# Audio-WestlakeU/FN-SSL

Measured on AMD Instinct MI355X. Metric: TF-frames/sec DP-IPD forward, 4-mic 257-bin x 300-frame, higher is better.
Workload: dtype f32; 1 GPU; BASELINE configs[1]: FN-SSL (online) DP-IPD forward, waveform->STFT->features->3x(full-band BiLSTM + narrow-band LSTM)->head; 32 utterances/GPU x 4 mics ('MM' = 6 pairs) x 257 bins x 300 frames, fp32; frame = one STFT frame of one utterance; stream_chunk_frames=0, utterances_per_gpu=32, global_batch=32, mics=4, pairs_per_utterance=6, frames=300, bins=257, parallelism=dp1 (utterance shards, no collective), chunk_pairs=0

## Files before the change

fn-ssl_amd/csrc/lstm_static4.h:

```cpp
#pragma once

#include "lstm_static.h"

#pragma clang fp contract(off)

namespace fnssl_lstm {

constexpr int static4_blocks_in_chunk(int qe, int chq, int nv0, int ns2, int ns) {
  int n = 0;
  for (int q = qe - chq + 1; q <= qe; ++q) {
    const bool x = q >= 1 && q <= nv0;
    const bool h = q >= 1 + nv0 + ns2 && q < 1 + nv0 + ns2 + ns;
    n += (x || h) ? 1 : 0;
  }
  return n;
}

template <int H, int NW, int NV0, int NS2, int CHQ, int PAD, int MODE, int XD = 4, bool PF4 = false>
__global__ void __launch_bounds__(NW * 64) lstm_static4_kernel(const LstmParams p) {
  FNSSL_GUARDED_KERNEL(p);
  constexpr int NS = H / 16, NP = NS / 4;
  constexpr int NB = NV0 + NS;
  constexpr bool HAS2 = (MODE & kHas2) != 0, SUM = (MODE & kSum) != 0;
  static_assert(!(MODE & kHas1) && HAS2 == (NS2 > 0) && NS % 4 == 0 && NS2 <= 1, "modes");
  constexpr int QPS = 1 + NV0 + NS2 + NS;
  constexpr int VQ = QPS + PAD;
  static_assert(VQ % CHQ == 0, "chunks must tile the (padded) slice quad");
  constexpr int CH = 16 * CHQ;
  constexpr int M = (CH + NW - 1) / NW;
  static_assert(PAD < CHQ, "a chunk of padding only would have no operand load to count the DMA by");
  extern __shared__ __attribute__((aligned(16))) char smem[];

  const WaveSeq<H, NW, 1, HAS2, SUM> pl(p);
  const int lane = pl.lane, w = pl.w;
  const rsrc_t rzero = __builtin_amdgcn_make_buffer_rsrc(const_cast<float*>(p.out), 0, 0, 0x00020000);

  const unsigned lds0 = (unsigned)(uintptr_t)smem;
  char* const lds_rd = smem + lane * 16;
  int dslot = 0, rslot = 0;
  int src_rec = 0;
  int src_vq = 0;
  auto issue_dma = [&]() {
#pragma unroll
    for (int m = 0; m < M; ++m) {
      const int r = w + m * NW;
      if (r < CH && src_vq * 16 + r < QPS * 16) {
        const unsigned soff = (unsigned)(src_rec + r) * 1024u;
        const unsigned ld = lds0 + (unsigned)(dslot * CH + r) * 1024u;
        asm volatile("s_mov_b32 m0, %2\n\ts_nop 0\n\tbuffer_load_dwordx4 %0, %1, %3 offen lds" ::"v"(pl.vlane), "s"(pl.rw),
                     "s"(__builtin_amdgcn_readfirstlane(ld)), "s"(__builtin_amdgcn_readfirstlane(soff))
                     : "memory");
      }
    }
    dslot ^= 1;
    src_vq += CHQ;
    src_rec += CH;
    if (src_vq == VQ) {
      src_vq = 0;
      src_rec -= PAD * 16;
      if (src_rec == NP * QPS * 16) src_rec = 0;
    }
  };
  issue_dma();
  asm volatile("s_waitcnt vmcnt(0)\n\ts_barrier" ::: "memory");
  issue_dma();
  const char* cb = lds_rd;
  auto rec = [&](auto ql, int j) { return *reinterpret_cast<const v4f*>(cb + decltype(ql)::value * 16384 + j * 1024); };
  v4f a0 = rec(ic<0>{}, 0), a1 = rec(ic<0>{}, 1);

  const v4f zero4 = v4f{0.f, 0.f, 0.f, 0.f};
  v4f acc[4][4];

  auto ring_step = [&](auto qi_c) {
    constexpr int QL = decltype(qi_c)::value % CHQ;
    if constexpr (QL + 1 < CHQ) {
      a0 = rec(ic<QL + 1>{}, 0);
      a1 = rec(ic<QL + 1>{}, 1);
    }
  };
  auto ring_end = [&](auto qi_c) {
    constexpr int QI = decltype(qi_c)::value, QL = QI % CHQ;
    if constexpr (QL + 1 == CHQ) {
      constexpr int K = static4_blocks_in_chunk(QI, CHQ, NV0, NS2, NS);
#ifdef FNSSL_BUILD_ABLATE
      asm volatile("s_waitcnt vmcnt(0)" ::: "memory");
#else
      if constexpr (K >= 3)
        asm volatile("s_waitcnt vmcnt(3)" ::: "memory");
      else if constexpr (K == 2)
        asm volatile("s_waitcnt vmcnt(2)" ::: "memory");
      else if constexpr (K == 1)
        asm volatile("s_waitcnt vmcnt(1)" ::: "memory");
      else
        asm volatile("s_waitcnt vmcnt(0)" ::: "memory");
#endif
      asm volatile("s_waitcnt lgkmcnt(0)\n\ts_barrier" ::: "memory");
      issue_dma();
      rslot ^= 1;
      cb = lds_rd + rslot * (CH * 1024);
      a0 = rec(ic<0>{}, 0);
      a1 = rec(ic<0>{}, 1);
    }
  };
#define SQUAD4(QI, B0, B1, B2, B3)                                                \
  do {                                                                            \
    const v4f a2_ = rec(ic<(QI) % CHQ>{}, 2), a3_ = rec(ic<(QI) % CHQ>{}, 3);     \
    __builtin_amdgcn_sched_barrier(0);                                            \
    MFMA4(acc[0], a0, B0);                                                        \
    MFMA4(acc[0], a1, B1);                                                        \
    const v4f b0_ = rec(ic<(QI) % CHQ>{}, 4), b1_ = rec(ic<(QI) % CHQ>{}, 5);     \
    __builtin_amdgcn_sched_barrier(0);                                            \
    MFMA4(acc[0], a2_, B2);                                                       \
    MFMA4(acc[0], a3_, B3);                                                       \
    const v4f b2_ = rec(ic<(QI) % CHQ>{}, 6), b3_ = rec(ic<(QI) % CHQ>{}, 7);     \
    __builtin_amdgcn_sched_barrier(0);                                            \
    MFMA4(acc[1], b0_, B0);                                                       \
    MFMA4(acc[1], b1_, B1);                                                       \
    const v4f c0_ = rec(ic<(QI) % CHQ>{}, 8), c1_ = rec(ic<(QI) % CHQ>{}, 9);     \
    __builtin_amdgcn_sched_barrier(0);                                            \
    MFMA4(acc[1], b2_, B2);                                                       \
    MFMA4(acc[1], b3_, B3);                                                       \
    const v4f c2_ = rec(ic<(QI) % CHQ>{}, 10), c3_ = rec(ic<(QI) % CHQ>{}, 11);   \
    __builtin_amdgcn_sched_barrier(0);                                            \
    MFMA4(acc[2], c0_, B0);                                                       \
    MFMA4(acc[2], c1_, B1);                                                       \
    const v4f d0_ = rec(ic<(QI) % CHQ>{}, 12), d1_ = rec(ic<(QI) % CHQ>{}, 13);   \
    __builtin_amdgcn_sched_barrier(0);                                            \
    MFMA4(acc[2], c2_, B2);                                                       \
    MFMA4(acc[2], c3_, B3);                                                       \
    const v4f d2_ = rec(ic<(QI) % CHQ>{}, 14), d3_ = rec(ic<(QI) % CHQ>{}, 15);   \
    __builtin_amdgcn_sched_barrier(0);                                            \
    MFMA4(acc[3], d0_, B0);                                                       \
    MFMA4(acc[3], d1_, B1);                                                       \
    ring_step(ic<(QI)>{});                                                        \
    __builtin_amdgcn_sched_barrier(0);                                            \
    MFMA4(acc[3], d2_, B2);                                                       \
    MFMA4(acc[3], d3_, B3);                                                       \
    ring_end(ic<(QI)>{});                                                         \
  } while (0)
#define SQUAD4_1(QI, B0)                                                                          \
  do {                                                                                            \
    const v4f b0_ = rec(ic<(QI) % CHQ>{}, 4), c0_ = rec(ic<(QI) % CHQ>{}, 8), d0_ = rec(ic<(QI) % CHQ>{}, 12); \
    MFMA4(acc[0], a0, B0);                                                                        \
    MFMA4(acc[1], b0_, B0);                                                                       \
    MFMA4(acc[2], c0_, B0);                                                                       \
    MFMA4(acc[3], d0_, B0);                                                                       \
    ring_step(ic<(QI)>{});                                                                        \
    ring_end(ic<(QI)>{});                                                                         \
  } while (0)

  OperandRing<XD, NV0, NS> ops;
  ops.prime(pl.rx0, pl.vo0, (pl.rev ? p.nsteps - 1 : 0) * pl.st0);

  for (int step = 0; step < p.nsteps; ++step) {
    const unsigned tt = pl.rev ? p.nsteps - 1 - step : step;
    const unsigned ttn = step + 1 < p.nsteps ? (pl.rev ? tt - 1 : tt + 1) : tt;
    const unsigned o0 = tt * pl.st0, o2 = tt * pl.st2, oo = tt * pl.sto, ok = tt * pl.stk;
    const unsigned op = (pl.rev ? tt + 1 : tt - 1) * pl.sto;
    const rsrc_t rh = step > 0 ? pl.ro : rzero;
    float xs2 = 0.f;
    if (NS2) xs2 = bld1(pl.rx2, pl.vo2, o2);

    for (int pr = 0; pr < NP; ++pr) {
      const int s0 = 4 * pr;
#ifdef FNSSL_BUILD_ABLATE
      const bool skip_ring = (p.ablate & 2) != 0;
#else
      constexpr bool skip_ring = false;
#endif
      v4f cprev = zero4, skipv = zero4;
      v4f cpf[PF4 ? 4 : 1], skf[PF4 ? 4 : 1];
      if constexpr (PF4) static_for<4>([&](auto s_) { cpf[s_.value] = zero4; skf[s_.value] = zero4; });
      const bool last = pr + 1 == NP;
      const unsigned nx = (last ? ttn : tt) * pl.st0;
      acc[0][0] = a0;
      acc[0][1] = a1;
      static_for<14>([&](auto j) {
        constexpr int J = decltype(j)::value + 2;
        acc[J / 4][J % 4] = rec(ic<0>{}, J);
      });
      ring_step(ic<0>{});
      ring_end(ic<0>{});
      static_for<NB>([&](auto bc) {
        constexpr int B = decltype(bc)::value;
        constexpr int QI = B < NV0 ? 1 + B : 1 + NS2 + B;
        if constexpr (NS2 > 0 && B == NV0) SQUAD4_1(1 + NV0, xs2);
        const v4f ob = ops.get(bc);
        if (!skip_ring) ops.request(bc, pl.rx0, pl.vo0, o0, nx, rh, pl.voo, op);
        if constexpr (!PF4 && B == NB - 4) {
          if (step > 0) cprev = bld4(pl.rc, pl.vlane, s0 * 1024);
          if (SUM) skipv = bld4(pl.rsk, pl.vok, ok + 64 * s0);
        }
        if constexpr (PF4 && B == NB - 3) {
          static_for<4>([&](auto s_) {
            constexpr int S = decltype(s_)::value;
            if (step > 0) cpf[S] = bld4(pl.rc, pl.vlane, (s0 + S) * 1024);
            if (SUM) skf[S] = bld4(pl.rsk, pl.vok, ok + 64 * (s0 + S));
          });
        }
        SQUAD4(QI, ob.x, ob.y, ob.z, ob.w);
      });
      static_for<PAD>([&](auto u) {
        ring_step(ic<QPS + decltype(u)::value>{});
        ring_end(ic<QPS + decltype(u)::value>{});
      });
      static_for<4>([&](auto sc) {
        constexpr int S = decltype(sc)::value;
        if constexpr (PF4) {
          cell_step(pl, acc[S], cpf[S], skf[S], (s0 + S) * 1024, oo + 64 * (s0 + S));
        } else {
          cell_step(pl, acc[S], cprev, skipv, (s0 + S) * 1024, oo + 64 * (s0 + S), [&] {
            if constexpr (S < 3) {
              if (step > 0) cprev = bld4(pl.rc, pl.vlane, (s0 + S + 1) * 1024);
              if (SUM) skipv = bld4(pl.rsk, pl.vok, ok + 64 * (s0 + S + 1));
            }
          });
        }
      });
    }
  }
  asm volatile("s_waitcnt vmcnt(0)" ::: "memory");
#undef SQUAD4
#undef SQUAD4_1
}

template <int H, int NW, int NV0, int NS2, int CHQ, int PAD, int MODE, int XD = 4, bool PF4 = false>
int launch_static4_k(const LstmParams& p, int nwg, const LaunchCtx& lc) {
  const size_t lds = (size_t)2 * CHQ * 16384;
  static_assert(2 * CHQ * 16384 <= 160 * 1024, "ring does not fit the LDS");
  return enqueue(lc, Kernel{lstm_static4_kernel<H, NW, NV0, NS2, CHQ, PAD, MODE, XD, PF4>, NW * 64, lds, "lstm_static4_kernel"}, nwg, p);
}

}
```

Baseline: 17780 frames/s.

## Interleave weight-ring DMA pieces between MFMA groups instead of bulk issue at chunk end

Instead of issuing all buffer_load-to-LDS pieces for the next weight chunk in one burst after the barrier, each piece is now placed at a compile-time-chosen MFMA group inside the first block quad of the current chunk. A constexpr schedule header computes piece placement and the matching vmcnt wait count per chunk, with static asserts to keep it consistent. Source and destination offsets become mostly compile-time with a wave-uniform base, and the step>0 branch on cell-state loads is replaced by a zero buffer descriptor. The intent is to hide DMA issue cost and spread memory traffic under MFMA work, at the risk of tighter wait counts and more scheduling constraints.

```diff
diff --git a/fn-ssl_amd/csrc/lstm_static4.h b/fn-ssl_amd/csrc/lstm_static4.h
--- a/fn-ssl_amd/csrc/lstm_static4.h
+++ b/fn-ssl_amd/csrc/lstm_static4.h
@@ -1,20 +1,11 @@
 #pragma once
 
 #include "lstm_static.h"
+#include "lstm_static4_sched.h"
 
 #pragma clang fp contract(off)
 
 namespace fnssl_lstm {
-
-constexpr int static4_blocks_in_chunk(int qe, int chq, int nv0, int ns2, int ns) {
-  int n = 0;
-  for (int q = qe - chq + 1; q <= qe; ++q) {
-    const bool x = q >= 1 && q <= nv0;
-    const bool h = q >= 1 + nv0 + ns2 && q < 1 + nv0 + ns2 + ns;
-    n += (x || h) ? 1 : 0;
-  }
-  return n;
-}
 
 template <int H, int NW, int NV0, int NS2, int CHQ, int PAD, int MODE, int XD = 4, bool PF4 = false>
 __global__ void __launch_bounds__(NW * 64) lstm_static4_kernel(const LstmParams p) {
@@ -29,6 +20,11 @@
   constexpr int CH = 16 * CHQ;
   constexpr int M = (CH + NW - 1) / NW;
   static_assert(PAD < CHQ, "a chunk of padding only would have no operand load to count the DMA by");
+  static_assert(M * NW == CH, "every wave issues every piece: the schedule has no wave-dependent piece");
+  constexpr Static4Shape SH{CHQ, NV0, NS2, NS, PAD, M};
+  constexpr int NC = VQ / CHQ;
+  static_assert(static4_schedule_ok(SH), "every chunk must place its M pieces and have a wait count");
+  constexpr unsigned SLOT = CH * 1024u;
   extern __shared__ __attribute__((aligned(16))) char smem[];
 
   const WaveSeq<H, NW, 1, HAS2, SUM> pl(p);
@@ -37,33 +33,35 @@
 
   const unsigned lds0 = (unsigned)(uintptr_t)smem;
   char* const lds_rd = smem + lane * 16;
-  int dslot = 0, rslot = 0;
-  int src_rec = 0;
-  int src_vq = 0;
-  auto issue_dma = [&]() {
-#pragma unroll
-    for (int m = 0; m < M; ++m) {
-      const int r = w + m * NW;
-      if (r < CH && src_vq * 16 + r < QPS * 16) {
-        const unsigned soff = (unsigned)(src_rec + r) * 1024u;
-        const unsigned ld = lds0 + (unsigned)(dslot * CH + r) * 1024u;
-        asm volatile("s_mov_b32 m0, %2\n\ts_nop 0\n\tbuffer_load_dwordx4 %0, %1, %3 offen lds" ::"v"(pl.vlane), "s"(pl.rw),
-                     "s"(__builtin_amdgcn_readfirstlane(ld)), "s"(__builtin_amdgcn_readfirstlane(soff))
-                     : "memory");
+  int rslot = 0;
+  const unsigned w_rec = (unsigned)w * 1024u;
+  constexpr unsigned PASS = QPS * 16384u;
+  auto dma_piece = [&](auto sc_c, auto m_c, unsigned src, unsigned dst) {
+    constexpr int SC = decltype(sc_c)::value, MI = decltype(m_c)::value;
+    constexpr int NVALID = static4_chunk_records(SH, SC);
+    if constexpr (MI * NW < NVALID) {
+      asm volatile("" : "+s"(src), "+s"(dst));
+      if constexpr (NVALID < MI * NW + NW) {
+        unsigned wc;
+        asm("s_min_u32 %0, %1, %2" : "=s"(wc) : "s"(w_rec), "s"((unsigned)(NVALID - 1 - MI * NW) * 1024u) : "scc");
+        src = src - w_rec + wc;
       }
-    }
-    dslot ^= 1;
-    src_vq += CHQ;
-    src_rec += CH;
-    if (src_vq == VQ) {
-      src_vq = 0;
-      src_rec -= PAD * 16;
-      if (src_rec == NP * QPS * 16) src_rec = 0;
-    }
-  };
-  issue_dma();
+      const unsigned soff = src + (unsigned)(SC * CH + MI * NW) * 1024u;
+      const unsigned ld = dst + (unsigned)(MI * NW) * 1024u;
+      const unsigned vl = pl.vlane;
+      const rsrc_t rw = pl.rw;
+#pragma clang diagnostic push
+#pragma clang diagnostic ignored "-Winline-asm"
+      asm volatile("s_mov_b32 m0, %2\n\ts_nop 0\n\tbuffer_load_dwordx4 %0, %1, %3 offen lds" ::"v"(vl), "s"(rw), "s"(ld), "s"(soff)
+                   : "memory", "m0");
+#pragma clang diagnostic pop
+    }
+  };
+  int ring_pr = 0;
+  auto src_cur = [&] { return (unsigned)ring_pr * PASS + w_rec; };
+  auto src_nxt = [&] { return (ring_pr + 1 < NP ? (unsigned)(ring_pr + 1) * PASS : 0u) + w_rec; };
+  static_for<M>([&](auto m_c) { dma_piece(ic<0>{}, m_c, w_rec, lds0 + w_rec); });
   asm volatile("s_waitcnt vmcnt(0)\n\ts_barrier" ::: "memory");
-  issue_dma();
   const char* cb = lds_rd;
   auto rec = [&](auto ql, int j) { return *reinterpret_cast<const v4f*>(cb + decltype(ql)::value * 16384 + j * 1024); };
   v4f a0 = rec(ic<0>{}, 0), a1 = rec(ic<0>{}, 1);
@@ -81,11 +79,12 @@
   auto ring_end = [&](auto qi_c) {
     constexpr int QI = decltype(qi_c)::value, QL = QI % CHQ;
     if constexpr (QL + 1 == CHQ) {
-      constexpr int K = static4_blocks_in_chunk(QI, CHQ, NV0, NS2, NS);
+      constexpr int C = QI / CHQ, K = static4_wait_count(SH, C);
+      static_assert(static4_pieces_placed(SH, C) == M && K >= 0 && K <= 3, "schedule");
 #ifdef FNSSL_BUILD_ABLATE
       asm volatile("s_waitcnt vmcnt(0)" ::: "memory");
 #else
-      if constexpr (K >= 3)
+      if constexpr (K == 3)
         asm volatile("s_waitcnt vmcnt(3)" ::: "memory");
       else if constexpr (K == 2)
         asm volatile("s_waitcnt vmcnt(2)" ::: "memory");
@@ -95,47 +94,60 @@
         asm volatile("s_waitcnt vmcnt(0)" ::: "memory");
 #endif
       asm volatile("s_waitcnt lgkmcnt(0)\n\ts_barrier" ::: "memory");
-      issue_dma();
       rslot ^= 1;
       cb = lds_rd + rslot * (CH * 1024);
       a0 = rec(ic<0>{}, 0);
       a1 = rec(ic<0>{}, 1);
     }
   };
+  auto ring_dma = [&](auto qi_c, auto g_c) {
+    constexpr int QI = decltype(qi_c)::value, C = QI / CHQ, MI = static4_piece_at(SH, QI, decltype(g_c)::value);
+    if constexpr (MI >= 0) {
+      dma_piece(ic<(C + 1) % NC>{}, ic<MI>{}, C + 1 < NC ? src_cur() : src_nxt(), lds0 + (unsigned)(rslot ^ 1) * SLOT + w_rec);
+    }
+  };
 #define SQUAD4(QI, B0, B1, B2, B3)                                                \
   do {                                                                            \
     const v4f a2_ = rec(ic<(QI) % CHQ>{}, 2), a3_ = rec(ic<(QI) % CHQ>{}, 3);     \
     __builtin_amdgcn_sched_barrier(0);                                            \
     MFMA4(acc[0], a0, B0);                                                        \
     MFMA4(acc[0], a1, B1);                                                        \
+    ring_dma(ic<(QI)>{}, ic<0>{});                                                \
     const v4f b0_ = rec(ic<(QI) % CHQ>{}, 4), b1_ = rec(ic<(QI) % CHQ>{}, 5);     \
     __builtin_amdgcn_sched_barrier(0);                                            \
     MFMA4(acc[0], a2_, B2);                                                       \
     MFMA4(acc[0], a3_, B3);                                                       \
+    ring_dma(ic<(QI)>{}, ic<1>{});                                                \
     const v4f b2_ = rec(ic<(QI) % CHQ>{}, 6), b3_ = rec(ic<(QI) % CHQ>{}, 7);     \
     __builtin_amdgcn_sched_barrier(0);                                            \
     MFMA4(acc[1], b0_, B0);                                                       \
     MFMA4(acc[1], b1_, B1);                                                       \
+    ring_dma(ic<(QI)>{}, ic<2>{});                                                \
     const v4f c0_ = rec(ic<(QI) % CHQ>{}, 8), c1_ = rec(ic<(QI) % CHQ>{}, 9);     \
     __builtin_amdgcn_sched_barrier(0);                                            \
     MFMA4(acc[1], b2_, B2);                                                       \
     MFMA4(acc[1], b3_, B3);                                                       \
+    ring_dma(ic<(QI)>{}, ic<3>{});                                                \
     const v4f c2_ = rec(ic<(QI) % CHQ>{}, 10), c3_ = rec(ic<(QI) % CHQ>{}, 11);   \
     __builtin_amdgcn_sched_barrier(0);                                            \
     MFMA4(acc[2], c0_, B0);                                                       \
     MFMA4(acc[2], c1_, B1);                                                       \
+    ring_dma(ic<(QI)>{}, ic<4>{});                                                \
     const v4f d0_ = rec(ic<(QI) % CHQ>{}, 12), d1_ = rec(ic<(QI) % CHQ>{}, 13);   \
     __builtin_amdgcn_sched_barrier(0);                                            \
     MFMA4(acc[2], c2_, B2);                                                       \
     MFMA4(acc[2], c3_, B3);                                                       \
+    ring_dma(ic<(QI)>{}, ic<5>{});                                                \
     const v4f d2_ = rec(ic<(QI) % CHQ>{}, 14), d3_ = rec(ic<(QI) % CHQ>{}, 15);   \
     __builtin_amdgcn_sched_barrier(0);                                            \
     MFMA4(acc[3], d0_, B0);                                                       \
     MFMA4(acc[3], d1_, B1);                                                       \
+    ring_dma(ic<(QI)>{}, ic<6>{});                                                \
     ring_step(ic<(QI)>{});                                                        \
     __builtin_amdgcn_sched_barrier(0);                                            \
     MFMA4(acc[3], d2_, B2);                                                       \
     MFMA4(acc[3], d3_, B3);                                                       \
+    ring_dma(ic<(QI)>{}, ic<7>{});                                                \
     ring_end(ic<(QI)>{});                                                         \
   } while (0)
 #define SQUAD4_1(QI, B0)                                                                          \
@@ -158,11 +170,13 @@
     const unsigned o0 = tt * pl.st0, o2 = tt * pl.st2, oo = tt * pl.sto, ok = tt * pl.stk;
     const unsigned op = (pl.rev ? tt + 1 : tt - 1) * pl.sto;
     const rsrc_t rh = step > 0 ? pl.ro : rzero;
+    const rsrc_t rcp = step > 0 ? pl.rc : rzero;
     float xs2 = 0.f;
     if (NS2) xs2 = bld1(pl.rx2, pl.vo2, o2);
 
     for (int pr = 0; pr < NP; ++pr) {
       const int s0 = 4 * pr;
+      ring_pr = pr;
 #ifdef FNSSL_BUILD_ABLATE
       const bool skip_ring = (p.ablate & 2) != 0;
 #else
@@ -188,13 +202,13 @@
         const v4f ob = ops.get(bc);
         if (!skip_ring) ops.request(bc, pl.rx0, pl.vo0, o0, nx, rh, pl.voo, op);
         if constexpr (!PF4 && B == NB - 4) {
-          if (step > 0) cprev = bld4(pl.rc, pl.vlane, s0 * 1024);
+          cprev = bld4(rcp, pl.vlane, s0 * 1024);
           if (SUM) skipv = bld4(pl.rsk, pl.vok, ok + 64 * s0);
         }
         if constexpr (PF4 && B == NB - 3) {
           static_for<4>([&](auto s_) {
             constexpr int S = decltype(s_)::value;
-            if (step > 0) cpf[S] = bld4(pl.rc, pl.vlane, (s0 + S) * 1024);
+            cpf[S] = bld4(rcp, pl.vlane, (s0 + S) * 1024);
             if (SUM) skf[S] = bld4(pl.rsk, pl.vok, ok + 64 * (s0 + S));
           });
         }
@@ -211,7 +225,7 @@
         } else {
           cell_step(pl, acc[S], cprev, skipv, (s0 + S) * 1024, oo + 64 * (s0 + S), [&] {
             if constexpr (S < 3) {
-              if (step > 0) cprev = bld4(pl.rc, pl.vlane, (s0 + S + 1) * 1024);
+              cprev = bld4(rcp, pl.vlane, (s0 + S + 1) * 1024);
               if (SUM) skipv = bld4(pl.rsk, pl.vok, ok + 64 * (s0 + S + 1));
             }
           });
diff --git a/fn-ssl_amd/csrc/lstm_static4_sched.h b/fn-ssl_amd/csrc/lstm_static4_sched.h
--- /dev/null
+++ b/fn-ssl_amd/csrc/lstm_static4_sched.h
@@ -0,0 +1,76 @@
+#pragma once
+
+namespace fnssl_lstm {
+
+constexpr int kStatic4Groups = 8;
+constexpr int kStatic4FirstGroup = 1;
+
+struct Static4Shape {
+  int chq, nv0, ns2, ns, pad, m;
+};
+
+constexpr int static4_qps(Static4Shape s) { return 1 + s.nv0 + s.ns2 + s.ns; }
+constexpr int static4_chunks(Static4Shape s) { return (static4_qps(s) + s.pad) / s.chq; }
+constexpr bool static4_is_block(Static4Shape s, int q) {
+  return (q >= 1 && q <= s.nv0) || (q >= 1 + s.nv0 + s.ns2 && q < static4_qps(s));
+}
+constexpr bool static4_has_mfma(Static4Shape s, int q) { return q >= 1 && q < static4_qps(s); }
+
+constexpr int static4_blocks_in_chunk(int qe, int chq, int nv0, int ns2, int ns) {
+  int n = 0;
+  for (int q = qe - chq + 1; q <= qe; ++q) n += static4_is_block(Static4Shape{chq, nv0, ns2, ns, 0, 0}, q) ? 1 : 0;
+  return n;
+}
+
+constexpr int static4_host_quad(Static4Shape s, int c) {
+  for (int q = c * s.chq; q < (c + 1) * s.chq; ++q)
+    if (static4_is_block(s, q)) return q;
+  return -1;
+}
+constexpr int static4_piece_stride(Static4Shape s, int c) {
+  const int h = static4_host_quad(s, c);
+  for (int q = h + 1; q < (c + 1) * s.chq; ++q)
+    if (static4_has_mfma(s, q)) return 2;
+  return 1;
+}
+struct Static4Pos {
+  int quad, group;
+};
+constexpr Static4Pos static4_piece_pos(Static4Shape s, int c, int m) {
+  const int h = static4_host_quad(s, c);
+  if (h < 0) return Static4Pos{-1, 0};
+  return Static4Pos{h, kStatic4FirstGroup + m * static4_piece_stride(s, c)};
+}
+constexpr int static4_piece_at(Static4Shape s, int q, int g) {
+  const int c = q / s.chq;
+  for (int m = 0; m < s.m; ++m) {
+    const Static4Pos p = static4_piece_pos(s, c, m);
+    if (p.quad == q && p.group == g) return m;
+  }
+  return -1;
+}
+constexpr int static4_pieces_placed(Static4Shape s, int c) {
+  int n = 0;
+  for (int q = c * s.chq; q < (c + 1) * s.chq; ++q)
+    if (static4_is_block(s, q))
+      for (int g = 0; g < kStatic4Groups; ++g) n += static4_piece_at(s, q, g) >= 0 ? 1 : 0;
+  return n;
+}
+constexpr int static4_wait_count(Static4Shape s, int c) {
+  const int last = static4_piece_pos(s, c, s.m - 1).quad;
+  if (last < 0) return -1;
+  int n = 0;
+  for (int q = c * s.chq; q < (c + 1) * s.chq; ++q) n += (q > last && static4_is_block(s, q)) ? 1 : 0;
+  return n;
+}
+constexpr bool static4_schedule_ok(Static4Shape s) {
+  for (int c = 0; c < static4_chunks(s); ++c)
+    if (static4_pieces_placed(s, c) != s.m || static4_wait_count(s, c) < 0) return false;
+  return true;
+}
+constexpr int static4_chunk_records(Static4Shape s, int sc) {
+  const int left = (static4_qps(s) - sc * s.chq) * 16;
+  return left < 16 * s.chq ? left : 16 * s.chq;
+}
+
+}
```

Result: no change. 17920 frames/s, median of 6 (+0.8%).
